# ExaScience/bpmf

Hardware: AMD Instinct MI355X
Metric: user+item column samples/sec per Gibbs iter; test RMSE vs reference (higher is better)
Workload: dtype f64

## Files before the change

### bpmf_amd/csrc/kernels.h

```cpp
#pragma once
#include <hip/hip_runtime.h>
#include <stdint.h>

#include "philox.h"
#include "args.h"

namespace bpmf {

typedef double d4 __attribute__((ext_vector_type(4)));

__device__ __forceinline__ d4 mfma16(double a, double b, d4 c)
{
    return __builtin_amdgcn_mfma_f64_16x16x4f64(a, b, c, 0, 0, 0);
}

__device__ __forceinline__ double mfma44(double a, double b, double c)
{
    return __builtin_amdgcn_mfma_f64_4x4x4f64(a, b, c, 0, 0, 0);
}

template <int K>
struct Rot44 {
    static constexpr int NT = K / 16;
    __host__ __device__ static constexpr int nrot(int TI, int TJ) { return TI == TJ ? 3 : 4; }
// ... 169 lines not shown
            out_lds[rank] = y * polar_mult(r2);
        }
        produced += __popcll(m);
        base += 64u;
    }
}

template <int NMAX>
__device__ __forceinline__ void draw_normals_deferred(uint32_t counter, int n, double *out_lds, double *r2_lds, int lane, int pad_to = 0)
{
    for (int i = n + lane; i < pad_to; i += 64) out_lds[i] = 0.0;
    int produced = 0;
    uint32_t base = 0;
    while (produced < n) {
        const Philox4 b = stream_block(counter, base + (uint32_t)lane);
        const double x = 2.0 * canonical53(b.w[3], b.w[2]) - 1.0;
        const double y = 2.0 * canonical53(b.w[1], b.w[0]) - 1.0;
        const double r2 = polar_r2(x, y);
        const bool acc = !(r2 > 1.0 || r2 == 0.0);
        const unsigned long long m = __ballot(acc);
        const int rank = produced + rank_below(m);
        if (acc && rank < n) { out_lds[rank] = y; r2_lds[rank] = r2; }
        produced += __popcll(m);
        base += 64u;
    }
    for (int i = lane; i < n; i += 64) {
        const double r2 = r2_lds[i];
        out_lds[i] = out_lds[i] * polar_mult(r2);
    }
}

template <int NMAX>
__device__ __forceinline__ void draw_normals_pair(uint32_t counterA, uint32_t counterB, int n, double *outA, double *outB,
                                                  double *r2A, double *r2B, int lane, int pad_to = 0)
{
    for (int i = n + lane; i < pad_to; i += 64) { outA[i] = 0.0; outB[i] = 0.0; }
    auto attempt = [&](uint32_t counter, uint32_t block, double &y, double &r2) -> bool {
        const Philox4 b = stream_block(counter, block);
        const double x = 2.0 * canonical53(b.w[3], b.w[2]) - 1.0;
        y = 2.0 * canonical53(b.w[1], b.w[0]) - 1.0;
        r2 = polar_r2(x, y);
        return !(r2 > 1.0 || r2 == 0.0);
    };
    int prodA, prodB;
    {
        double y, r2;
        bool acc = attempt(counterA, (uint32_t)lane, y, r2);
        unsigned long long m = __ballot(acc);
        int rank = rank_below(m);
        if (acc && rank < n) { outA[rank] = y; r2A[rank] = r2; }
        prodA = __popcll(m);
        acc = attempt(counterB, (uint32_t)lane, y, r2);
        m = __ballot(acc);
        rank = rank_below(m);
        if (acc && rank < n) { outB[rank] = y; r2B[rank] = r2; }
        prodB = __popcll(m);
    }
    const bool hi = lane >= 32;
    const int l32 = lane & 31;
    uint32_t base = 64u;
    while (prodA < n || prodB < n) {
        double y, r2;
        const bool acc = attempt(hi ? counterB : counterA, base + (uint32_t)l32, y, r2);
        const unsigned long long m = __ballot(acc);
        const unsigned mA = (unsigned)m, mB = (unsigned)(m >> 32);
        const int rank = hi ? prodB + (int)__builtin_amdgcn_mbcnt_hi(mB, 0u) : prodA + (int)__builtin_amdgcn_mbcnt_lo(mA, 0u);
        if (acc && rank < n) { (hi ? outB : outA)[rank] = y; (hi ? r2B : r2A)[rank] = r2; }
        prodA += __popc(mA); prodB += __popc(mB);
        base += 32u;
    }
    for (int i = lane; i < n; i += 64) {
        const double ra = r2A[i], rb = r2B[i];
        outA[i] = outA[i] * polar_mult(ra);
        outB[i] = outB[i] * polar_mult(rb);
    }
}

template <int K>
__device__ __forceinline__ void gram_chunk(const int32_t *__restrict__ rowidx, const double *__restrict__ vals, int len,
                                           const double *__restrict__ other, const double *__restrict__ zero_row, double mean, double alpha,
                                           d4 (&acc)[Geo<K>::NTRI], double (&r)[Geo<K>::NT], int lane, int rowmask = -1)
{
    constexpr int NT = Geo<K>::NT;
    const int kq = lane >> 4, li = lane & 15;
    int ri_n = (0 + lane < len) ? rowidx[lane] : -1;
    double wv_n = (0 + lane < len) ? (vals[lane] - mean) * alpha : 0.0;
    for (int b = 0; b < len; b += 64) {
        const int ri = ri_n;
        const double wv = wv_n;
        if (b + 64 < len) {
            const int q = b + 64 + lane;
            ri_n = (q < len) ? rowidx[q] : -1;
            wv_n = (q < len) ? (vals[q] - mean) * alpha : 0.0;
        }
        const int nsteps = (len - b >= 64) ? 16 : (len - b + 3) >> 2;
        double y[4][NT], w[4];
        auto gather = [&](int g, double (&yy)[4][NT], double (&ww)[4]) {
#pragma unroll
            for (int s = 0; s < 4; ++s) {
                const int src = (g * 4 + s) * 4 + kq;
                const int row = __shfl(ri, src);
                ww[s] = __shfl(wv, src);
                const double *col = (row >= 0) ? other + (size_t)(row & rowmask) * K : zero_row;
#pragma unroll
                for (int t = 0; t < NT; ++t) yy[s][t] = col[(t * 16 + li < K) ? t * 16 + li : 0];
            }
        };
        gather(0, y, w);
#pragma unroll
        for (int g = 0; g < 4; ++g) {
            if (g * 4 >= nsteps) break;
            double yn[4][NT], wn[4];
            const bool more = (g + 1) * 4 < nsteps;
            if (g < 3 && more) gather(g + 1, yn, wn);
#pragma unroll
            for (int s = 0; s < 4; ++s) {
#pragma unroll
                for (int t = 0; t < NT; ++t) r[t] = fma(y[s][t], w[s], r[t]);
                int tri = 0;
#pragma unroll
                for (int I = 0; I < NT; ++I)
#pragma unroll
                    for (int J = I; J < NT; ++J, ++tri) acc[tri] = mfma16(y[s][I], y[s][J], acc[tri]);
            }
            if (g < 3 && more) {
#pragma unroll
                for (int s = 0; s < 4; ++s) {
                    w[s] = wn[s];
#pragma unroll
                    for (int t = 0; t < NT; ++t) y[s][t] = yn[s][t];
                }
            }
        }
    }
#pragma unroll
    for (int t = 0; t < NT; ++t) {
        r[t] += __shfl_xor(r[t], 16);
        r[t] += __shfl_xor(r[t], 32);
    }
}

template <int CTRL>
__device__ __forceinline__ double row_ror_add(double x)
{
    const long long v = __builtin_bit_cast(long long, x);
    const int lo = (int)v, hi = (int)(v >> 32);
    const int rlo = __builtin_amdgcn_update_dpp(0, lo, CTRL, 0xF, 0xF, true);
    const int rhi = __builtin_amdgcn_update_dpp(0, hi, CTRL, 0xF, 0xF, true);
    const long long rv = ((long long)rhi << 32) | (unsigned int)rlo;
    return x + __builtin_bit_cast(double, rv);
}

template <bool WT> struct IdxBlockT { int ri; double v; int base; };
template <> struct IdxBlockT<true> { int ri; double v; int base; double s; };
typedef IdxBlockT<false> IdxBlock;
template <bool WT = false>
__device__ __forceinline__ IdxBlockT<WT> load_idx_block(const int32_t *__restrict__ rowidx, const double *__restrict__ vals, int base, int lane, int len,
                                                        const double *__restrict__ safe, const double *__restrict__ sw = nullptr)
{
    IdxBlockT<WT> r;
    const int q = base + lane;
    const int32_t *pr = (q < len) ? rowidx + q : reinterpret_cast<const int32_t *>(safe);
    const double *pv = (q < len) ? vals + q : safe;
    r.ri = *pr;
    r.v = *pv;
    if constexpr (WT) {
        const double *ps = (q < len) ? sw + q : safe;
        r.s = *ps;
    }
    r.base = base;
    return r;
}

template <int K, bool WT = false>
__device__ __forceinline__ void gram_chunk44(const int32_t *__restrict__ rowidx, const double *__restrict__ vals, int len,
                                             const double *__restrict__ other, const double *__restrict__ zero_row,
                                             double mean, double alpha, IdxBlockT<WT> cur, IdxBlockT<WT> nxt,
                                             double (&acc)[Geo44<K>::NB], double (&rr)[Geo44<K>::NG], int lane, int rowmask = -1,
                                             const double *__restrict__ sw = nullptr)
{
    using G = Geo44<K>;
    constexpr int NG = G::NG, NL = G::NL;
    typedef double dd2 __attribute__((ext_vector_type(2)));
    const int slot = lane >> 2, x = lane & 3;
    auto gather = [&](const IdxBlockT<WT> &ib, int gg, dd2 (&yy)[NL], double &ww, double &ss) {
        const int src = gg * 16 + slot;
        const int row = __shfl(ib.ri, src);
        ww = (__shfl(ib.v, src) - mean) * alpha;
        if constexpr (WT) ss = __shfl(ib.s, src);
        const double *base = (ib.base + src < len) ? other + (size_t)(row & rowmask) * K : zero_row;
        const dd2 *p = reinterpret_cast<const dd2 *>(base + 2 * x);
#pragma unroll
        for (int h = 0; h < NL; ++h) yy[h] = p[4 * h];
    };
    auto contract = [&](const dd2 (&yy)[NL], double ww, double ss) {
        double R[NG];
#pragma unroll
        for (int h = 0; h < NL; ++h) { R[2 * h] = yy[h].x; R[2 * h + 1] = yy[h].y; }
        if constexpr (WT) {
#pragma unroll
            for (int g = 0; g < NG; ++g) R[g] *= ss;
        }
#pragma unroll
        for (int g = 0; g < NG; ++g) rr[g] = fma(R[g], ww, rr[g]);
        int blk = 0;
#pragma unroll
        for (int g = 0; g < NG; ++g)
#pragma unroll
            for (int g2 = g; g2 < NG; ++g2, ++blk) acc[blk] = mfma44(R[g], R[g2], acc[blk]);
    };
    if (len <= 0) return;
    dd2 yA[NL], yB[NL];
    double wA, wB = 0.0, sA = 0.0, sB = 0.0;
    gather(cur, 0, yA, wA, sA);
    int b0 = 0;
    for (; b0 + 64 < len; b0 += 64) {
        IdxBlockT<WT> nn{};
        if constexpr (!WT) nn = load_idx_block<WT>(rowidx, vals, b0 + 128, lane, len, zero_row, sw);
        gather(cur, 1, yB, wB, sB);
        contract(yA, wA, sA);
        gather(cur, 2, yA, wA, sA);
        contract(yB, wB, sB);
        gather(cur, 3, yB, wB, sB);
        contract(yA, wA, sA);
        gather(nxt, 0, yA, wA, sA);
        contract(yB, wB, sB);
        cur = nxt;
        if constexpr (WT) nxt = load_idx_block<WT>(rowidx, vals, b0 + 128, lane, len, zero_row, sw);
        else nxt = nn;
    }
    const int ng = (len - b0 + 15) >> 4;
    if (ng > 1) gather(cur, 1, yB, wB, sB);
    contract(yA, wA, sA);
    if (ng > 1) {
        if (ng > 2) gather(cur, 2, yA, wA, sA);
        contract(yB, wB, sB);
        if (ng > 2) {
            if (ng > 3) gather(cur, 3, yB, wB, sB);
            contract(yA, wA, sA);
            if (ng > 3) contract(yB, wB, sB);
        }
    }
}

typedef double gs_raw __attribute__((ext_vector_type(2)));
__device__ __forceinline__ gs_raw load_gs_rec(const GatherRec *__restrict__ rec, int g, unsigned slot_bytes)
{
    return *reinterpret_cast<const gs_raw *>(reinterpret_cast<const char *>(rec + 16 * g) + slot_bytes);
}

template <int K>
__device__ __forceinline__ void gram_stream44(const GatherRec *__restrict__ rec, int ng, const double *__restrict__ other,
                                              const double *__restrict__ zero_row, double alpha, gs_raw r0, gs_raw r1, unsigned slot_bytes,
                                              double (&acc)[Geo44<K>::NB], double (&rr)[Geo44<K>::NG], int lane)
{
    using G = Geo44<K>;
    constexpr int NG = G::NG, NL = G::NL;
    typedef double dd2 __attribute__((ext_vector_type(2)));
    const int x = lane & 3;
    const dd2 *ox = reinterpret_cast<const dd2 *>(other + 2 * x), *zx = reinterpret_cast<const dd2 *>(zero_row + 2 * x);
    auto gather = [&](const gs_raw &rc, dd2 (&yy)[NL], double &ww) {
        const int off = (int)__builtin_bit_cast(long long, rc.x);
        ww = rc.y * alpha;
        const dd2 *p = (off >= 0) ? ox + off : zx;
#pragma unroll
        for (int h = 0; h < NL; ++h) yy[h] = p[4 * h];
    };
    auto contract = [&](const dd2 (&yy)[NL], double ww) {
        double R[NG];
#pragma unroll
        for (int h = 0; h < NL; ++h) { R[2 * h] = yy[h].x; R[2 * h + 1] = yy[h].y; }
#pragma unroll
        for (int g = 0; g < NG; ++g) rr[g] = fma(R[g], ww, rr[g]);
        int blk = 0;
#pragma unroll
        for (int g = 0; g < NG; ++g)
#pragma unroll
            for (int g2 = g; g2 < NG; ++g2, ++blk) acc[blk] = mfma44(R[g], R[g2], acc[blk]);
    };
    if (ng <= 0) return;
    dd2 yA[NL], yB[NL];
    double wA, wB = 0.0;
    gather(r0, yA, wA);
    r0 = load_gs_rec(rec, 2, slot_bytes);
    if (ng > 1) gather(r1, yB, wB);
    r1 = load_gs_rec(rec, 3, slot_bytes);
    contract(yA, wA);
    int g = 1;
    for (; g + 2 < ng; g += 2) {
        gather(r0, yA, wA);
        r0 = load_gs_rec(rec, g + 3, slot_bytes);
        contract(yB, wB);
        gather(r1, yB, wB);
        r1 = load_gs_rec(rec, g + 4, slot_bytes);
        contract(yA, wA);
    }
    if (g < ng) {
        if (g + 1 < ng) gather(r0, yA, wA);
        contract(yB, wB);
        if (g + 1 < ng) contract(yA, wA);
    }
}

template <int K>
__device__ __forceinline__ void assemble44(double (&acc)[Geo44<K>::NB], double (&rr)[Geo44<K>::NG], double *sA, double *sb,
                                           int LD, int lane)
{
    using G = Geo44<K>;
    constexpr int NG = G::NG;
    static_assert(NG % 2 == 0, "block rows are written in pairs");
    const int i = lane >> 4, b = (lane >> 2) & 3, j = lane & 3;
    auto blk = [](int g, int g2) constexpr { return g * NG - (g * (g - 1)) / 2 + (g2 - g); };
    double *up = sA + (2 * i) * LD + 2 * j;
    double *lo = sA + (2 * j) * LD + 2 * i;
#pragma unroll
    for (int g = 0; g < NG; g += 2) {
#pragma unroll
        for (int t = blk(g, g); t < blk(g + 1, NG - 1) + 1; ++t) {
            const double v = row_ror_add<0x128>(acc[t]);
            acc[t] = row_ror_add<0x124>(v);
        }
        if (b == 0) {
            up[G::idx(g + 1, 0) * LD + G::idx(g + 1, 0)] = acc[blk(g + 1, g + 1)];
#pragma unroll
            for (int g2 = g; g2 < NG; g2 += 2) {
                double2 v; v.x = acc[blk(g, g2)]; v.y = acc[blk(g, g2 + 1)];
                *reinterpret_cast<double2 *>(&up[G::idx(g, 0) * LD + G::idx(g2, 0)]) = v;
                if (g2 > g) {
                    double2 w; w.x = acc[blk(g + 1, g2)]; w.y = acc[blk(g + 1, g2 + 1)];
                    *reinterpret_cast<double2 *>(&up[G::idx(g + 1, 0) * LD + G::idx(g2, 0)]) = w;
                }
            }
        } else if (b == 1) {
            lo[G::idx(g + 1, 0) * LD + G::idx(g, 0)] = acc[blk(g, g + 1)];
#pragma unroll
            for (int g2 = g + 2; g2 < NG; ++g2) {
                double2 v; v.x = acc[blk(g, g2)]; v.y = acc[blk(g + 1, g2)];
                *reinterpret_cast<double2 *>(&lo[G::idx(g2, 0) * LD + G::idx(g, 0)]) = v;
            }
        }
    }
#pragma unroll
    for (int g = 0; g < NG; ++g) {
        double v = row_ror_add<0x128>(rr[g]);
        v = row_ror_add<0x124>(v);
        v += __shfl_xor(v, 16);
        v += __shfl_xor(v, 32);
        if (lane < 4) sb[G::idx(g, lane)] = v;
    }
}

template <int K>
__device__ __forceinline__ void deposit_column(const SampleArgs &a, int64_t idx, const d4 (&acc)[Geo<K>::NTRI],
                                               const double (&r)[Geo<K>::NT], double *lds, int slot, int lane)
{
    using G = Geo<K>;
    constexpr int NT = G::NT;
    const int kq = lane >> 4, li = lane & 15;
    double *sL = lds + slot * G::SLOT, *sY = sL + G::PLEN, *sZ = sY + K;

    draw_normals<K>(sample_counter(idx, a.ktrue, a.iter_plus_1), a.ktrue, sZ, lane, K);
    const double *LF = a.prop_lambda ? a.prop_lambda + (size_t)(idx - a.col_from) * K * K : a.LambdaF;

    int tri = 0;
#pragma unroll
    for (int I = 0; I < NT; ++I)
#pragma unroll
        for (int J = I; J < NT; ++J, ++tri)
#pragma unroll
            for (int reg = 0; reg < 4; ++reg) {
                const int gi = I * 16 + kq + 4 * reg, gj = J * 16 + li;
                const int row = (I == J) ? gi : gj, col = (I == J) ? gj : gi;
                if (row < K && col <= row)
                    sL[tri_off(row) + col] = (a.diag_only && row != col) ? 0.0 : fma(a.alpha, acc[tri][reg], LF[row + col * K]);
            }
    if (kq == 0) {
#pragma unroll
        for (int t = 0; t < NT; ++t)
            if (t * 16 + li < K) {
                double lm = a.Lmu[t * 16 + li];
                if (a.prop_lambda) {
                    lm = 0.0;
                    for (int j = 0; j < K; ++j) lm = fma(LF[t * 16 + li + j * K], a.mu[j], lm);
                }
                sY[t * 16 + li] = lm + r[t];
            }
    }
    if (lane == 0) reinterpret_cast<long long *>(lds + G::C * G::SLOT)[slot] = idx;
}

template <int K>
struct Pivot { double dinv0, dinv1, l10; };

template <int K>
__device__ __forceinline__ Pivot<K> factor_block(double pa, double pb, double pc)
{
    Pivot<K> v;
    v.dinv0 = rsqrt_nr(pa);
    const double rdet = rsqrt_nr(fma(pa, pc, -(pb * pb)));
    v.dinv1 = rdet * (pa * v.dinv0);
    v.l10 = pb * v.dinv0;
    return v;
}

template <int K>
__device__ __forceinline__ void finish_slots(const SampleArgs &a, double *lds, int nfilled, int lane_in)
{
    using G = Geo<K>;
    constexpr int NP = G::NP;
    int lane = lane_in;
    asm volatile("" : "+v"(lane));
    const int c = lane / K, i = lane % K;
    double *sL = lds + c * G::SLOT, *sY = sL + G::PLEN, *sZ = sY + K;
    double *myrow = sL + tri_off(i);
    const int gbase = 4 * (c * K);
    __syncthreads();

    double row[K + 1];
#pragma unroll
    for (int j = 0; j < K; j += 2) {
        const double2 g = *reinterpret_cast<const double2 *>(&myrow[j]);
        row[j] = g.x;
        row[j + 1] = g.y;
    }
    row[K] = sY[i];
    const double zi = sZ[i];
    Pivot<K> pv = factor_block<K>(sL[0], sL[tri_off(1)], sL[tri_off(1) + 1]);
    __syncthreads();

#pragma unroll
    for (int p = 0; p < NP; ++p) {
        const int k = 2 * p;
        double2 lp;
        lp.x = row[k] * pv.dinv0;
        lp.y = fma(-lp.x, pv.l10, row[k + 1]) * pv.dinv1;
        if (i >= k) *reinterpret_cast<double2 *>(&myrow[k]) = lp;

        double na = 0.0, nb = 0.0, nc = 0.0;
        if (p + 1 < NP) {
            na = gbcast(row[k + 2], gbase, k + 2);
            nb = gbcast(row[k + 2], gbase, k + 3);
            nc = gbcast(row[k + 3], gbase, k + 3);
        }
        const double rb0 = gbcast(row[K], gbase, k), rb1 = gbcast(row[K], gbase, k + 1);
        __syncthreads();
        const double2 L = *reinterpret_cast<const double2 *>(&myrow[k]);
        Pivot<K> pn = pv;
        if (p + 1 < NP) {
            const double2 l0 = *reinterpret_cast<const double2 *>(&sL[tri_off(k + 2) + k]);
            const double2 l1 = *reinterpret_cast<const double2 *>(&sL[tri_off(k + 3) + k]);
            const double pa = fma(-l0.y, l0.y, fma(-l0.x, l0.x, na));
            const double pb = fma(-l1.y, l0.y, fma(-l1.x, l0.x, nb));
            const double pc = fma(-l1.y, l1.y, fma(-l1.x, l1.x, nc));
            pn = factor_block<K>(pa, pb, pc);
        }
        const double yk = rb0 * pv.dinv0;
        const double yk1 = fma(-pv.l10, yk, rb1) * pv.dinv1;
        if (i == 0) *reinterpret_cast<double2 *>(&sY[k]) = double2{yk, yk1};
        row[K] = fma(-L.y, yk1, fma(-L.x, yk, row[K]));
#pragma unroll
        for (int j = k + 2; j < K; ++j) {
            const double2 A = *reinterpret_cast<const double2 *>(&sL[tri_off(j) + k]);
            row[j] = fma(-L.y, A.y, fma(-L.x, A.x, row[j]));
        }
#pragma unroll
        for (int m = k + 2; m < K + 1; ++m) asm volatile("" : "+v"(row[m]));
        pv = pn;
    }
    __syncthreads();

    double bi = sY[i] + zi;
    const double my_dinv = 1.0 / myrow[i];
    constexpr int BB = K < 8 ? K : 8;
#pragma unroll
    for (int kb = K - BB; kb >= 0; kb -= BB) {
        double lv[BB];
#pragma unroll
        for (int t = 0; t < BB; ++t) lv[t] = sL[tri_off(kb + t) + i];
#pragma unroll
        for (int t = BB - 1; t >= 0; --t) {
            const int k = kb + t;
            if (k == 0) continue;
            const double xk = gbcast(bi * my_dinv, gbase, k);
            bi = (i < k) ? fma(-lv[t], xk, bi) : bi;
        }
    }
    const double xi = bi * my_dinv;

    if (c < nfilled) {
        const long long idx = reinterpret_cast<const long long *>(lds + G::C * G::SLOT)[c];
        a.items[(size_t)idx * K + i] = xi;
        if (!(fabs(xi) <= 1.79769313486231570815e+308)) atomicMin(a.fail, (unsigned long long)idx);
    }
    __syncthreads();
}

#define BPMF_RLX_AGENT __ATOMIC_RELAXED, __HIP_MEMORY_SCOPE_AGENT

template <int K>
struct Geo1 {
    static constexpr int S = (64 / K < K / 2) ? 64 / K : K / 2;
    static constexpr int NP = K / 2;
    static constexpr int QN = NP / S;
    static constexpr int M = 2 * QN;
    static constexpr int FLD = K + 2;
    static constexpr bool PACKED = K == 64;
    __host__ __device__ static constexpr int roff_c(int j) { return (j & 1) ? ((j + 1) * (j + 1)) / 2 : (j * (j + 2)) / 2; }
    static constexpr int AWORDS = PACKED ? roff_c(K) : K * FLD;
    static constexpr int LANES = K * S;
    static constexpr int LDS_WORDS = AWORDS + 4 * K + 2;
    static constexpr int WPS = K == 32 ? 3 : (K < 32 ? 4 : 2);
};

template <int K, typename Assemble>
__device__ __forceinline__ void finish_single(const SampleArgs &a, int col_local, double *lds, int lane_in, bool have_z,
                                              Assemble &&assemble)
{
    int lane = lane_in;
    using G = Geo1<K>;
    constexpr int LD = G::FLD, S = G::S, NP = G::NP, QN = G::QN, M = G::M;
    asm volatile("" : "+v"(lane));
    double *sA = lds, *sb = lds + G::AWORDS, *sz = sb + K, *sdummy = sz + K, *szero = sdummy + 2 * K;
    auto roff = [](int j) -> int {
        if constexpr (G::PACKED) return (j & 1) ? ((j + 1) * (j + 1)) >> 1 : (j * (j + 2)) >> 1;
        else return j * G::FLD;
    };
    const int64_t idx = a.col_from + col_local;

    if (!have_z) draw_normals<K>(sample_counter(idx, a.ktrue, a.iter_plus_1), a.ktrue, sz, lane, K);

    const int l = lane & (G::LANES - 1);
    const int h = l / K, i = l % K;
    const double *LF = a.prop_lambda ? a.prop_lambda + (size_t)col_local * K * K : a.LambdaF;
    constexpr bool PRELOAD = K <= 32;
    double lf[PRELOAD ? M : 2];
    if constexpr (PRELOAD) {
#pragma unroll
        for (int q = 0; q < QN; ++q) {
            const int j = 2 * (q * S + h);
            lf[2 * q] = LF[i + j * K];
            lf[2 * q + 1] = LF[i + (j + 1) * K];
        }
    }
    double lmu = a.Lmu[i];
    if (a.prop_lambda) {
        lmu = 0.0;
        for (int j = 0; j < K; ++j) lmu = fma(LF[i + j * K], a.mu[j], lmu);
    }

    assemble(sA, sb, LD, lane);
    if (lane < 2) szero[lane] = 0.0;
    __syncthreads();

    double row[M + 2];
#pragma unroll
    for (int q = 0; q < QN; ++q) {
        double2 g;
        if constexpr (G::PACKED) {
            const int j = 2 * (q * S + h);
            g.x = sA[(j <= i) ? roff(i) + j : roff(j) + i];
            g.y = sA[(j + 1 <= i) ? roff(i) + j + 1 : roff(j + 1) + i];
        } else {
            g = *reinterpret_cast<const double2 *>(&sA[i * LD + 2 * (q * S + h)]);
        }
        if constexpr (PRELOAD) {
            row[2 * q] = fma(a.alpha, g.x, lf[2 * q]);
            row[2 * q + 1] = fma(a.alpha, g.y, lf[2 * q + 1]);
        } else {
            const int j = 2 * (q * S + h);
            row[2 * q] = fma(a.alpha, g.x, LF[i + j * K]);
            row[2 * q + 1] = fma(a.alpha, g.y, LF[i + (j + 1) * K]);
        }
    }
    if (a.diag_only) {
#pragma unroll
        for (int q = 0; q < QN; ++q) {
            const int j = 2 * (q * S + h);
            row[2 * q] = (j == i) ? row[2 * q] : 0.0;
            row[2 * q + 1] = (j + 1 == i) ? row[2 * q + 1] : 0.0;
        }
    }
    row[M] = (h == 0) ? lmu + sb[i] : 0.0;
    row[M + 1] = 0.0;
    const double zi = sz[i];
    double yi = 0.0;
    __syncthreads();

#pragma unroll
    for (int p = 0; p < NP; ++p) {
        const int hk = p % S, qk = p / S, k = 2 * p;
        const int src0 = hk * K + k, src1 = src0 + 1;
        const double pa = bcast(row[2 * qk], src0);
        const double pb = bcast(row[2 * qk], src1);
        const double pc = bcast(row[2 * qk + 1], src1);
        const double bk = bcast(row[M], k), bk1 = bcast(row[M], k + 1);
        const double dinv0 = rsqrt_nr(pa);
        const double rdet = rsqrt_nr(fma(pa, pc, -(pb * pb)));
        const double dinv1 = rdet * (pa * dinv0);
        const double l10 = pb * dinv0;
        const double yk = bk * dinv0;
        const double yk1 = fma(-l10, yk, bk1) * dinv1;
        yi = (i == k) ? yk : yi;
        yi = (i == k + 1) ? yk1 : yi;
        double2 lp;
        lp.x = row[2 * qk] * dinv0;
        lp.y = fma(-lp.x, l10, row[2 * qk + 1]) * dinv1;
        double *dst = (h == hk && (!G::PACKED || i >= k)) ? &sA[roff(i) + k] : &sdummy[2 * i];
        *reinterpret_cast<double2 *>(dst) = lp;
        __syncthreads();
        const double2 L = *reinterpret_cast<const double2 *>((!G::PACKED || i >= k) ? &sA[roff(i) + k] : szero);
// ... 680 lines not shown
```

Baseline: 105.8 million.

## Pack cross-bank reductions with DPP merges in K=32 normal-equation assembly

For K=32, the MFMA 4x4 accumulator reduction and store is replaced by a packed scheme. Four independent block accumulators are merged across DPP banks so that each lane ends up holding a distinct final sum, rather than every lane reducing each block separately. The right-hand-side reduction uses permlane16/32 swaps. This aims to cut the number of cross-lane reduction instructions and the branch-guarded stores, at the cost of intricate index mapping that must match the layout exactly.

```diff
diff --git a/bpmf_amd/csrc/kernels.h b/bpmf_amd/csrc/kernels.h
--- a/bpmf_amd/csrc/kernels.h
+++ b/bpmf_amd/csrc/kernels.h
@@ -495,10 +495,100 @@
     }
 }
 
+template <int CTRL, int BANKS>
+__device__ __forceinline__ double dpp_merge(double old, double src)
+{
+    const long long o = __builtin_bit_cast(long long, old), v = __builtin_bit_cast(long long, src);
+    const int lo = __builtin_amdgcn_update_dpp((int)o, (int)v, CTRL, 0xF, BANKS, false);
+    const int hi = __builtin_amdgcn_update_dpp((int)(o >> 32), (int)(v >> 32), CTRL, 0xF, BANKS, false);
+    return __builtin_bit_cast(double, ((long long)hi << 32) | (unsigned int)lo);
+}
+
+__device__ __forceinline__ double bank_totals4(double x0, double x1, double y0, double y1)
+{
+    const double u0 = dpp_merge<0x128, 0x3>(y0, x0), v0 = dpp_merge<0x128, 0xC>(x0, y0);
+    const double z0 = v0 + u0;
+    const double u1 = dpp_merge<0x128, 0x3>(y1, x1), v1 = dpp_merge<0x128, 0xC>(x1, y1);
+    const double z1 = v1 + u1;
+    const double p = dpp_merge<0x12C, 0x5>(z1, z0), q = dpp_merge<0x124, 0xA>(z0, z1);
+    return q + p;
+}
+
+template <bool WIDE>
+__device__ __forceinline__ double row_swap_add(double x, double y)
+{
+    const unsigned long long a = __builtin_bit_cast(unsigned long long, x), b = __builtin_bit_cast(unsigned long long, y);
+    unsigned alo, blo, ahi, bhi;
+    if constexpr (WIDE) {
+        const auto l = __builtin_amdgcn_permlane32_swap((unsigned)a, (unsigned)b, false, false);
+        const auto h = __builtin_amdgcn_permlane32_swap((unsigned)(a >> 32), (unsigned)(b >> 32), false, false);
+        alo = l[0]; blo = l[1]; ahi = h[0]; bhi = h[1];
+    } else {
+        const auto l = __builtin_amdgcn_permlane16_swap((unsigned)a, (unsigned)b, false, false);
+        const auto h = __builtin_amdgcn_permlane16_swap((unsigned)(a >> 32), (unsigned)(b >> 32), false, false);
+        alo = l[0]; blo = l[1]; ahi = h[0]; bhi = h[1];
+    }
+    return __builtin_bit_cast(double, ((unsigned long long)ahi << 32) | alo) + __builtin_bit_cast(double, ((unsigned long long)bhi << 32) | blo);
+}
+
+template <int K>
+__device__ __forceinline__ void assemble44_packed(double (&acc)[Geo44<K>::NB], double (&rr)[Geo44<K>::NG], double *sA, double *sb,
+                                                  int LD, int lane)
+{
+    using G = Geo44<K>;
+    constexpr int NG = G::NG;
+    static_assert(NG == 8, "the packing is the one of K = 32");
+    const int i = lane >> 4, b = (lane >> 2) & 3, j = lane & 3;
+    auto blk = [](int g, int g2) constexpr { return g * NG - (g * (g - 1)) / 2 + (g2 - g); };
+    const int ib = G::idx(b, 0), b1 = b & 1;
+    const int quad = (b >> 1) * (G::idx(4, 0) * LD + G::idx(4, 0));
+    double *up = sA + (2 * i) * LD + 2 * j;
+    double *lo = sA + (2 * j) * LD + 2 * i;
+    {
+        double *pu = up + quad + b1, *pl = lo + quad + b1 * LD;
+#pragma unroll
+        for (int g = 0; g < 2; ++g) {
+            const double v = bank_totals4(acc[blk(g, 2)], acc[blk(g, 3)], acc[blk(g + 4, 6)], acc[blk(g + 4, 7)]);
+            pu[G::idx(g, 0) * LD + G::idx(2, 0)] = v;
+            pl[G::idx(2, 0) * LD + G::idx(g, 0)] = v;
+        }
+        const int d = b1 * (G::idx(2, 0) * LD + G::idx(2, 0));
+        const double v = bank_totals4(acc[blk(0, 1)], acc[blk(2, 3)], acc[blk(4, 5)], acc[blk(6, 7)]);
+        up[quad + d + G::idx(0, 0) * LD + G::idx(1, 0)] = v;
+        lo[quad + d + G::idx(1, 0) * LD + G::idx(0, 0)] = v;
+    }
+    {
+        double *pu = up + ib, *pl = lo + ib * LD;
+#pragma unroll
+        for (int g = 0; g < 4; ++g) {
+            const double v = bank_totals4(acc[blk(g, 4)], acc[blk(g, 5)], acc[blk(g, 6)], acc[blk(g, 7)]);
+            pu[G::idx(g, 0) * LD + G::idx(4, 0)] = v;
+            pl[G::idx(4, 0) * LD + G::idx(g, 0)] = v;
+        }
+    }
+    {
+        double *p = up + ib * (LD + 1);
+#pragma unroll
+        for (int h = 0; h < 2; ++h)
+            p[G::idx(4 * h, 0) * (LD + 1)] = bank_totals4(acc[blk(4 * h, 4 * h)], acc[blk(4 * h + 1, 4 * h + 1)],
+                                                          acc[blk(4 * h + 2, 4 * h + 2)], acc[blk(4 * h + 3, 4 * h + 3)]);
+    }
+    {
+        const double w0 = bank_totals4(rr[0], rr[1], rr[2], rr[3]), w1 = bank_totals4(rr[4], rr[5], rr[6], rr[7]);
+        const double s = row_swap_add<false>(w0, w1);
+        const double t = row_swap_add<true>(s, s);
+        sb[G::idx(4 * (i & 1), 0) + G::idx(b, j)] = t;
+    }
+}
+
 template <int K>
 __device__ __forceinline__ void assemble44(double (&acc)[Geo44<K>::NB], double (&rr)[Geo44<K>::NG], double *sA, double *sb,
                                            int LD, int lane)
 {
+    if constexpr (K == 32) {
+        assemble44_packed<K>(acc, rr, sA, sb, LD, lane);
+        return;
+    }
     using G = Geo44<K>;
     constexpr int NG = G::NG;
     static_assert(NG % 2 == 0, "block rows are written in pairs");
```

New measurement: 111.7 million (median of 6 runs). 1.06x the previous value.
